# magnusgrandin/ca-lanczos

Hardware: AMD Instinct MI355X
Metric: CA-Lanczos outer-iters/sec (n~10M, s=8) (higher is better)
Workload: dtype f64; 1 GPU; lap3d_215: 7-pt 3-D 215x..., n=9938375, nnz=69291275; s=8, basis=newton, orth=local, parallelism=row-slab x1, normalize=auto, comm=none, halo=none

## Files before the change

ca_lanczos_amd/csrc/blockorth.cpp:

```cpp
#include <algorithm>
#include <chrono>
#include <cstdlib>
#include <cmath>
#include <vector>

#include "cal_internal.hpp"
#include "comm.hpp"
#include "dense.hpp"

namespace cal {

static Panel panel_slice(const Panel& P, int c0, int nc) {
    Panel out = panel();
    int base = 0;
    for (int s = 0; s < P.nseg; ++s) {
        const int lo = std::max(c0, base), hi = std::min(c0 + nc, base + P.ncol[s]);
        if (hi > lo) panel_add(out, P.ptr[s] + (int64_t)(lo - base) * P.ld[s], P.ld[s], hi - lo);
        base += P.ncol[s];
    }
    return out;
}

static PanelOut panel_out_slice(const PanelOut& P, int c0, int nc) {
    PanelOut out{};
// ... 297 lines not shown
    auto coeffs_b = [&](bool* sh2) -> int {
        std::vector<double> Gp = G1, Rb((size_t)m * m), Rbi((size_t)m * m);
        for (int j = 0; j < m; ++j)
            for (int i = 0; i < m; ++i) {
                double s = 0.0;
                for (int k = 0; k < w; ++k) s += C3[k + (size_t)i * w] * C3[k + (size_t)j * w];
                Gp[i + (size_t)j * m] -= s;
            }
        if (!chol_or_shift(m, Gp.data(), ng, Rb.data(), sh2))
            return set_error(c, CAL_ERR_NUMERIC, "block orthogonalisation: second Cholesky failed");
        dense::tri_inv_upper(m, Rb.data(), m, Rbi.data(), m);
        std::fill(M2.begin(), M2.end(), 0.0);
        for (int j = 0; j < m; ++j) {
            for (int i = 0; i < w; ++i) {
                double s = 0.0;
                for (int k = 0; k <= j; ++k) s += C3[i + (size_t)k * w] * Rbi[k + (size_t)j * m];
                M2[i + (size_t)j * (w + m)] = -s;
            }
            for (int i = 0; i < m; ++i) M2[w + i + (size_t)j * (w + m)] = Rbi[i + (size_t)j * m];
        }
        for (int j = 0; j < m; ++j)
            for (int i = 0; i < w; ++i) {
                double s = 0.0;
                for (int k = 0; k <= j; ++k) s += C3[i + (size_t)k * w] * Racc[k + (size_t)j * m];
                Ctot[i + (size_t)j * w] += s;
            }
        std::vector<double> Rn((size_t)m * m, 0.0);
        dense::matmul(m, m, m, Rb.data(), m, Racc.data(), m, Rn.data(), m);
        for (int j = 0; j < m; ++j)
            for (int i = j + 1; i < m; ++i) Rn[i + (size_t)j * m] = 0.0;
        Racc = Rn;
        return 0;
    };
    if (fast && !sh) {
        double G16[256], e16[16];
        CAL_TRY(rowapply_host(c, n, W, M1.data(), m, Qout, 2, w, G16, e16));
        unpack(G16, e16, G1, C3);
        bool sh2 = false;
        CAL_TRY(coeffs_b(&sh2));
        CAL_TRY(rowapply_host(c, n, W, M1.data(), m, Qout, 3, w, nullptr, nullptr, M2.data()));
        std::copy(Racc.begin(), Racc.end(), R);
        *shifted = *shifted || sh2;
        return 0;
    }
    CAL_TRY(grams(W, M1, G1, C3, false));
    const int passes = sh ? 2 : 1;
    for (int p = 0; p < passes; ++p) {
        bool sh2 = false;
        CAL_TRY(coeffs_b(&sh2));
        sh = sh || sh2;
        const bool more = p + 1 < passes;
        CAL_TRY(grams(P2, M2, G1, C3, !more));
    }
    std::copy(Racc.begin(), Racc.end(), R);
    *shifted = *shifted || sh;
    return 0;
}

static bool orth_device_ok(cal_ctx* c, const Panel& Qp, const Panel& X) {
    const int w = Qp.total, m = X.total, nq = w < 8 ? w : 8;
    return c->orth_coef_device && m >= 1 && w <= 9 && nq + m <= 16 && Qp.nseg + X.nseg <= kMaxSeg &&
           rowapply_ok(w + m, m, true, w);
}

constexpr int kSweepResMax = 3;
constexpr int64_t kSweepResBudget = ((int64_t)256 << 20) / 32 * 29;
static int sweep_policy(cal_ctx* c, int64_t n, int w, int m) {
    int res = -1;
    if (w == 9 && m == 8 && !c->pbw.want && !test_switch("CAL_TEST_SWEEP_STREAM_OFF")) {
        const int64_t r = std::min<int64_t>(std::min(m, kSweepResMax), kSweepResBudget / (8 * std::max<int64_t>(n, 1)));
        const bool large = (int64_t)n * 8 * (w + m) > ((int64_t)256 << 20);
        if ((large && c->sweep_x_fresh) || test_switch("CAL_TEST_SWEEP_STREAM_ON")) res = (int)r;
    }
#ifdef CAL_TEST_HOOKS
    c->test_sweep_res = res;
#endif
    return res;
}

#ifdef CAL_TEST_HOOKS
}
extern "C" int cal_test_sweep_policy(cal_ctx* c) { return c ? c->test_sweep_res : -2; }
extern "C" int cal_test_sweep_coef(cal_ctx* c) { return c ? c->test_sweep_coef : -2; }
namespace cal {
#endif

static int wait_published(cal_ctx* c, const unsigned long long* h_seq, unsigned long long seq) {
    const auto t0 = std::chrono::steady_clock::now();
    for (uint64_t spin = 1;; ++spin) {
        if (__atomic_load_n(h_seq, __ATOMIC_ACQUIRE) == seq) return 0;
        if ((spin & 4095) == 0 && std::chrono::steady_clock::now() - t0 > std::chrono::seconds(2)) {
            CAL_HIP(c, hipStreamSynchronize(c->stream));
            if (__atomic_load_n(h_seq, __ATOMIC_ACQUIRE) == seq) return 0;
            return set_error(c, CAL_ERR_HIP, "block orthogonalisation: result never published");
        }
        __builtin_ia32_pause();
    }
}

static int orth_device(cal_ctx* c, int64_t n, const Panel& Qp, const Panel& X, bool doreorth, const PanelOut& Qout,
                       double* Rq, double* R, bool* reorth, int p1_blocks = 0) {
    const int w = Qp.total, m = X.total, nq = w < 8 ? w : 8, wp = w + m;
    const int WP = rowapply_wpmax(wp), MO = rowapply_mout(m);
    const Panel W = panel_concat(Qp, X);
    const int res = sweep_policy(c, n, w, m);
    const int csrc = test_switch("CAL_TEST_SWEEP_COEF_LDS") ? 0 : (test_switch("CAL_TEST_SWEEP_COEF_SCALAR") ? 1 : -1);
#ifdef CAL_TEST_HOOKS
    c->test_sweep_coef = rowapply_coef(wp, m, 2, n, csrc);
#endif
    CAL_TRY(ensure_red(c, 4096));
    double* d_tile = c->d_red;
    double* d_st = c->d_red + 1024;
    double* d_mbuf = c->d_red + 2048;
    double* d_out = c->d_red + 3072;
#ifdef CAL_TEST_HOOKS
    CAL_HIP(c, hipMemsetAsync(c->d_red, 0xFF, 4096 * sizeof(double), c->stream));
#endif
    const double* gate = test_switch("CAL_TEST_NO_PASSB_GATE") ? nullptr : d_out + 512;
    const int64_t rg_cap = (int64_t)n * 8 * 17 <= ((int64_t)160 << 20) ? kRowGramBlocks / 2 : kRowGramBlocks;
    int64_t blocks = std::max<int64_t>(1, std::min<int64_t>((n + 255) / 256, rg_cap));
    CAL_TRY(ensure_partial(c, (size_t)blocks * 272));
    ColList ct{};
    if (p1_blocks > 0 && w == 0) {
    } else {
        p1_blocks = 0;
        const Panel T = panel_concat(panel_slice(W, 0, nq), X);
        const int nt = T.total;
        for (int cc = 0; cc < 16; ++cc) ct.p[cc] = panel_slice(T, cc < nt ? cc : nt - 1, 1).ptr[0];
        ct.p[16] = w == 9 ? panel_slice(Qp, 8, 1).ptr[0] : ct.p[0];
        const int t = timer_begin(c, 1, 8.0 * n * (nt + (w == 9 ? 1 : 0)));
        CAL_HIP(c, launch_rowgram(ct, nt, w == 9, n, (int)blocks, c->d_partial, c->stream, res));
        timer_end(c, t);
    }
    CAL_TRY(ensure_pub(c));
    const unsigned long long seq = ++c->pub_seq;
    double* h_out = c->h_pub;
    unsigned long long* h_seq = reinterpret_cast<unsigned long long*>(c->h_pub + 516);
    unsigned long long* d_seq = reinterpret_cast<unsigned long long*>(c->d_pub + 516);
    auto coef = [&](int phase, int dore) -> int {
        const int np = phase == 0 && p1_blocks > 0 ? p1_blocks : (int)blocks;
        CAL_HIP_OTHER(c, launch_reduce(c->d_partial, np, 272, d_tile, c->stream));
        CAL_TRY(allreduce_sum(c, d_tile, 272));
        CAL_HIP_OTHER(c, launch_orth_coef(phase, d_tile, d_st, d_mbuf, d_out, w, m, WP, MO, dore,
                                    phase == 1 ? c->d_pub : nullptr, d_seq, seq, c->stream));
        return 0;
    };
    CAL_TRY(coef(0, doreorth ? 1 : 0));
    ColList cw{};
    OutList ol{};
    for (int cc = 0; cc < 17; ++cc) cw.p[cc] = panel_slice(W, cc < wp ? cc : wp - 1, 1).ptr[0];
    for (int j = 0; j < 16; ++j) ol.p[j] = panel_out_slice(Qout, j < m ? j : 0, 1).ptr[0];
    {
        const int t = timer_begin(c, 1, 8.0 * n * wp);
        CAL_HIP(c, launch_rowapply(cw, d_mbuf, wp, m, ol, 2, w, n, (int)blocks, c->d_partial, c->stream, nullptr,
                                   res, csrc));
        timer_end(c, t);
    }
    CAL_TRY(coef(1, 0));
    const bool pbw = c->pbw.want && w == 9 && m == 8 && WP == 17 && MO == 8 &&
                     passb_wide_tiles(c->pbw.qold.total) <= kPassbWideMaxTiles && Qp.nseg == 1 &&
                     c->pbw.qold.nseg <= 1;
    c->pbw.want = false;
    c->pbw.ready = false;
    if (pbw) {
        const int ntw = passb_wide_tiles(c->pbw.qold.total);
        const size_t ent = (size_t)128 * ntw;
        const int pblocks = (int)std::max<int64_t>(1, std::min<int64_t>((n + 255) / 256, kRowGramBlocks));
        CAL_TRY(ensure_partial(c, (size_t)pblocks * ent));
        if (ent > c->pbw.cap) {
            if (c->pbw.d) CAL_HIP(c, hipFree(c->pbw.d));
            if (c->pbw.h) CAL_HIP(c, hipHostFree(c->pbw.h));
            c->pbw.d = c->pbw.h = nullptr;
            c->pbw.cap = 0;
            const size_t cap = (size_t)128 * kPassbWideMaxTiles;
            CAL_HIP(c, scratch_malloc((void**)&c->pbw.d, cap * sizeof(double)));
            CAL_HIP(c, hipHostMalloc((void**)&c->pbw.h, cap * sizeof(double), hipHostMallocDefault));
            c->pbw.cap = cap;
        }
        if (!c->pbw.ev) CAL_HIP(c, hipEventCreateWithFlags(&c->pbw.ev, hipEventDisableTiming));
        const int t = timer_begin(c, 2, 8.0 * n * (wp + m + c->pbw.qold.total));
        CAL_HIP(c, launch_passb_wide(cw, d_mbuf, ol, c->pbw.qold, n, pblocks, c->d_partial, gate, c->stream));
        timer_end(c, t);
        CAL_HIP_OTHER(c, launch_reduce(c->d_partial, pblocks, (int64_t)ent, c->pbw.d, c->stream));
        CAL_TRY(allreduce_sum(c, c->pbw.d, (int64_t)ent));
        CAL_HIP_OTHER(c, hipMemcpyAsync(c->pbw.h, c->pbw.d, ent * sizeof(double), hipMemcpyDeviceToHost, c->stream));
        CAL_HIP(c, hipEventRecord(c->pbw.ev, c->stream));
        c->pbw.ntw = ntw;
    } else {
        const int t = timer_begin(c, 2, 8.0 * n * (wp + m));
        CAL_HIP(c, launch_rowapply(cw, d_mbuf, wp, m, ol, 3, w, n, (int)((n + 255) / 256), c->d_partial, c->stream,
                                   gate, res, csrc));
        timer_end(c, t);
    }
    if (c->pre_wait) {
        auto hook = std::move(c->pre_wait);
        c->pre_wait = nullptr;
        CAL_TRY(hook());
    }
    CAL_TRY(wait_published(c, h_seq, seq));
    if (h_out[512] != 0.0 || h_out[513] != 0.0) return 1;
    c->pbw.ready = pbw;
    std::copy(h_out, h_out + (size_t)m * m, R);
    std::copy(h_out + 256, h_out + 256 + (size_t)w * m, Rq);
    *reorth = h_out[514] != 0.0;
    return 0;
}

int normalize_dev(cal_ctx* c, int64_t n, const Panel& X, const PanelOut& Qout, double* R, double tol, int* rank,
                  bool* shifted, int p1_blocks) {
    const int m = X.total;
    if (use_tsqr(c, m, c->tier1)) {
        CAL_TRY(tsqr_dev(c, n, X, nullptr, m, Qout, R));
        if (shifted) *shifted = false;
        if (rank) *rank = rank_from_R(m, R, tol);
        return 0;
    }
    auto via_tsqr = [&]() -> int {
        CAL_TRY(tsqr_dev(c, n, X, nullptr, m, Qout, R));
        if (shifted) *shifted = false;
        if (rank) *rank = rank_from_R(m, R, tol);
        return 0;
    };
    if (m > 16 && tsqr_ok(m)) return via_tsqr();
    if (m < 1 || m > 16) return set_error(c, CAL_ERR_ARG, "normalize: 1..32 columns supported");
    if (orth_device_ok(c, panel(), X)) {
        bool ro = false;
        const int st = orth_device(c, n, panel(), X, false, Qout, nullptr, R, &ro, p1_blocks);
        CAL_TRY(st);
        if (st == 0) {
            if (shifted) *shifted = false;
            if (rank) *rank = rank_from_R(m, R, tol);
            return 0;
        }
        c->orth_redone = true;
        if (c->normalize_kind != 2) return via_tsqr();
    }
    std::vector<double> G((size_t)m * m), Mz((size_t)m * m, 0.0), Ctot;
    if (X.nseg <= kMaxSeg) {
// ... 706 lines not shown
```

ca_lanczos_amd/csrc/cal_internal.hpp:

```cpp
#pragma once

#include <hip/hip_runtime.h>
#include <rocprofiler-sdk-roctx/roctx.h>

#include <cstdint>
#include <cstdlib>
#include <functional>
#include <string>
#include <vector>

#include "../../include/calanczos.h"

struct RoctxRange {
    explicit RoctxRange(const char* msg) { roctxRangePushA(msg); }
    ~RoctxRange() { roctxRangePop(); }
    RoctxRange(const RoctxRange&) = delete;
    RoctxRange& operator=(const RoctxRange&) = delete;
};

namespace cal {

constexpr int kMaxSeg = 4;

struct Panel {
// ... 147 lines not shown
    bool ds_neg1 = false;
    uint8_t* ds_rowmask = nullptr;
    uint32_t* ds_wavemask = nullptr;
    double* ds_diag = nullptr;
    double* ds_gsum = nullptr;
    double* ds_dprod = nullptr;
    bool shared = false;
    int64_t n_half = 0;
    bool herm = false;
    double* vim = nullptr;
    int* dpos = nullptr;
    int dpos_state = 0;
    int64_t dpos_missing = 0, dpos_dup = 0;
    std::vector<int> peers;
    std::vector<int64_t> recv_off;
    std::vector<int64_t> recv_cnt;
    std::vector<int64_t> send_off;
    std::vector<int64_t> send_cnt;
    int* send_idx = nullptr;
    int64_t send_total = 0;
    double* send_buf = nullptr;
};

struct Comm;
struct LanczosState;
struct PropState;
struct StdLanczosState;

hipError_t launch_spmv(const SpmvArgs& a, hipStream_t st);
hipError_t launch_spmv_stacked(const SpmvArgs& a, const double* vim, int64_t n_half, hipStream_t st);
hipError_t launch_spmv_pat(const PatArgs& a, hipStream_t st);
int spmv_lanczos_blocks(const SpmvArgs& a);
int spmv_pat_lanczos_blocks(const PatArgs& a);
hipError_t launch_spmv_dsplit(const PatArgs& a, hipStream_t st);
int spmv_dsplit_blocks(const PatArgs& a);
struct GramPlan {
    int nta;
    int blocks;
    int64_t entries;
};
GramPlan gram_plan(int wa, int wb, int64_t n);
hipError_t launch_gram(const Panel& A, const Panel& B, int64_t n, const GramPlan& pl, double* partial,
                       hipStream_t st);
bool gram_bb_ok(int wa, int wb);
hipError_t launch_gram_bb(const Panel& A, const Panel& B, int64_t n, const GramPlan& pl, double* partial,
                          hipStream_t st);
struct ApplyPlan {
    int nty;
    int run;
    int blocks;
    bool gram;
    bool gramp;
    size_t lds_bytes;
    int64_t entries;
};
ApplyPlan apply_plan(int wp, int wy, int64_t n, bool gram, int wq);
int apply_rows_max_wy(int wp);
bool apply_rows_ok(int wp, int wy);
bool apply_gram_ok(int wp, int wy, int wq);
int apply_gram_blocks(int64_t n);
hipError_t launch_apply_gram(const Panel& P, const double* dM, int wp, int wy, const PanelOut& Y, const Panel& Qn,
                             int64_t n, double* partial, hipStream_t st);
bool apply_selfgram_ok(int wp, int wy);
hipError_t launch_apply_selfgram(const Panel& P, const double* dM, int wp, int wy, const PanelOut& Y, int64_t n,
                                 double* partial, int* blocks, hipStream_t st);
hipError_t launch_apply(const Panel& P, const double* dM, int wp, int wy, const PanelOut& Y, bool store,
                        int wq, int64_t n, const ApplyPlan& pl, double* partial, hipStream_t st);
hipError_t launch_reduce(const double* partial, int nparts, int64_t nent, double* out, hipStream_t st);
hipError_t launch_gram_wide(const double* Q, int64_t ld, int w, int64_t n, double* partial, hipStream_t st);
int gram_wide_entries(int w);
int gram_wide_blocks(int64_t n);
void gram_wide_entry(int w, int e, int* i, int* j);
hipError_t launch_tilegram(const Panel& T, const double* E, int64_t n, int blocks, double* partial, hipStream_t st);
int rowapply_wpmax(int wp);
int rowapply_mout(int m);
struct ColList {
    const double* p[17];
};
struct OutList {
    double* p[16];
};
hipError_t launch_rowapply(const ColList& P, const double* dM, int wp, int m, const OutList& Y, int kind, int wq,
                           int64_t n, int blocks, double* partial, hipStream_t st, const double* gate = nullptr,
                           int res = -1, int coef = -1);
int rowapply_coef(int wp, int m, int kind, int64_t n, int coef);
hipError_t launch_orth_coef(int phase, const double* tile, double* st, double* mbuf, double* out, int w, int m,
                            int WP, int MO, int doreorth, double* hout, unsigned long long* hseq,
                            unsigned long long seq, hipStream_t stream);
#ifndef CAL_ROWGRAM_BLOCKS
#define CAL_ROWGRAM_BLOCKS 1024
#endif
constexpr int kRowGramBlocks = CAL_ROWGRAM_BLOCKS;
hipError_t launch_rowgram(const ColList& P, int nt, bool has_extra, int64_t n, int blocks, double* partial,
                          hipStream_t st, int res = -1);
constexpr int kPassbWideMaxTiles = 12;
int passb_wide_tiles(int wold);
hipError_t launch_passb_wide(const ColList& P, const double* dM, const OutList& Y, const Panel& Qold, int64_t n,
                             int blocks, double* partial, const double* gate, hipStream_t st);
hipError_t launch_dot(const double* x, const double* y, int64_t n, double* partial, int blocks,
                      hipStream_t st);
int dot_blocks(int64_t n);
hipError_t launch_axpy_sub(double* y, const double* x, double a, int64_t n, hipStream_t st);
hipError_t launch_div(double* y, const double* x, double b, int64_t n, hipStream_t st);
hipError_t launch_form_projM(const double* G, int ldg, int w, int m, double* M, hipStream_t st);
hipError_t launch_normest_norms(double* x, const double* y, int64_t n, double* part, double* dst, hipStream_t st);
hipError_t launch_normest_norms_only(const double* x, const double* y, int64_t n, double* part, double* dst,
                                     hipStream_t st);
hipError_t launch_pro_step(double* r, const double* qprev, const double* pb_prev, const double* q, double* qnext,
                           int64_t n, double* part, double* d_alpha, double* d_beta2, hipStream_t st);
hipError_t launch_pro_tail(double* r, const double* q, double* qnext, int64_t n, const double* pa, int np, double* pb,
                           double* d_alpha, double* d_beta2, hipStream_t st);
hipError_t launch_axpy_sub_dev(double* y, const double* x, const double* pa, bool take_sqrt, int64_t n,
                               hipStream_t st);
hipError_t launch_div_sqrt(double* y, const double* x, const double* nn, int64_t n, hipStream_t st);
hipError_t launch_abs_rowsum(const int* rowptr, const double* val, int64_t n, double* y, hipStream_t st);
hipError_t launch_gather(double* dst, const double* src, const int* idx, int64_t cnt, hipStream_t st);
int gram_async(cal_ctx* c, int64_t n, const Panel& A, const Panel& B, double* d_dst, double* h_dst, int* ldc,
               double* part = nullptr, bool bb = false);
int spmv_pair_resid_blocks(const PatArgs& a);
hipError_t launch_spmv_pair_resid(const PatArgs& a, double lr, double* partial, hipStream_t st);
hipError_t launch_spmv_pair_resid_multi(const PatArgs& a, const double* X, int64_t ldx, const int* col,
                                        const double* lam, const int* out, int npr, double* partial,
                                        int64_t pstride, hipStream_t st);
int spmv_resid_pair_multi_dev(cal_ctx* c, const double* X, int64_t ldx, const int* col, const double* lam,
                              const int* out, int npr, double* partial, int64_t pstride);
int spmv_pair_resid_multi_blocks(const PatArgs& a);
int spmv_resid_pair_multi_blocks(cal_ctx* c);
bool apply_mt_ok(int wp, int wy);
hipError_t launch_apply_mt(const double* P, int64_t ldp, const double* dM, int wp, int wy, double* Y, int64_t ldy,
                           int64_t n, hipStream_t st);
int spmv_resid_pair_dev(cal_ctx* c, const double* x, double lr, double* partial, int* blocks);
int spmv_resid_pair_blocks(cal_ctx* c);
hipError_t launch_spmv_resid(const SpmvArgs& a, const double* xi, double lr, double li, int64_t nrows,
                             double* partial, int blocks, hipStream_t st);

constexpr int kTsqrMaxCols = 33;
struct TsqrCols {
    const double* p[kTsqrMaxCols];
};
struct TsqrQ {
    double* p[32];
};
struct TsqrLevelArgs {
    int64_t rows = 0;
    int m = 0;
    int wp = 0;
    const double* M = nullptr;
    const double* in = nullptr;
    double* out = nullptr;
    const double* S = nullptr;
    const double* M2 = nullptr;
    int w2 = 0;
    double* V = nullptr;
    double* tb = nullptr;
};
int tsqr_mm(int m);
int tsqr_tile_rows(int m);
bool tsqr_form_ok(int wp, int m);
hipError_t launch_tsqr(bool down, int src, const TsqrLevelArgs& a, const TsqrCols& P, const TsqrQ& Q,
                       hipStream_t st);


constexpr double kFoldTol = 1e-14;
struct FoldArgs {
    int64_t n = 0;
    double tol = kFoldTol;
    int m = 0, w = 0, nblk = 0, n0 = 0, nlev = 0;
    int nu[3] = {0, 0, 0};
    const double* C = nullptr;
    const double* flags = nullptr;
    const double* K = nullptr;
    double *V0 = nullptr, *tb0 = nullptr, *R0 = nullptr;
    double* Vu[3] = {nullptr, nullptr, nullptr};
    double* Ru[3] = {nullptr, nullptr, nullptr};
    double* Mu[3] = {nullptr, nullptr, nullptr};
    double* Rroot_m = nullptr;
    double* partial = nullptr;
// ... 78 lines not shown
    hipEvent_t a, b;
    double bytes;
};

struct cal_ctx {
    int device = 0;
    hipStream_t stream = nullptr;
    hipStream_t aux_stream = nullptr;
    std::string err;
    cal::DevMatrix A;
    bool has_A = false;
    uint64_t A_gen = 0;
    int64_t stat_spmv_rows = 0;

    double* d_partial = nullptr;
    size_t partial_cap = 0;
    double* d_red = nullptr;
    double* h_red = nullptr;
    size_t red_cap = 0;
    double* d_small = nullptr;
    double* h_small = nullptr;
    size_t small_cap = 0;
    bool small_pending = false;
    double* d_scratch = nullptr;
    size_t scratch_cap = 0;

    double* d_work = nullptr;
    int work_cols = 0;
    int64_t work_ld = 0;

    cal::LanczosState* lz = nullptr;
    cal::PropState* prop = nullptr;
    cal::StdLanczosState* slz = nullptr;
    cal::Comm* comm = nullptr;

    bool timing = false;
    std::vector<CalTimerRec> timers;
    std::vector<hipEvent_t> event_pool;

    int spmv_format = 0;
    int mpk_depth_req = 8;
    int powers_launches = 0;
    int powers_schedule = -1;
    bool orth_coef_device = true;
    std::function<int()> pre_wait;
    struct {
        bool want = false, ready = false;
        cal::Panel qold{};
        int ntw = 0;
        double* d = nullptr;
        double* h = nullptr;
        size_t cap = 0;
        hipEvent_t ev = nullptr;
    } pbw;
    bool orth_redone = false;
    bool sweep_x_fresh = false;
    hipEvent_t orth_event = nullptr;
    double* h_pub = nullptr;
    double* d_pub = nullptr;
    unsigned long long pub_seq = 0;
    int normalize_kind = 0;
    bool tier1 = false;
    double* d_tsqr = nullptr;
    size_t tsqr_cap = 0;
    double* d_tsqrv = nullptr;
    size_t tsqrv_cap = 0;
    double* d_zbuf = nullptr;
    size_t zbuf_cap = 0;
    double* d_fold = nullptr;
    size_t fold_cap = 0;
    long fold_runs = 0, fold_declined = 0;
    double fold_last_est = 0.0;
    double fold_tol = cal::kFoldTol;
    hipStream_t nest_stream = nullptr;
    hipEvent_t nest_event = nullptr;
    double* d_nest = nullptr;
    double* h_nest = nullptr;
    size_t nest_cap = 0;
    hipGraphExec_t nest_exec[2] = {nullptr, nullptr};
    std::vector<int64_t> nest_key[2];
    std::vector<double> test_R1;
    int test_sweep_res = -2;
    int test_sweep_coef = -2;
};

namespace cal {

int set_error(cal_ctx* c, int code, const std::string& msg);
int hip_fail(cal_ctx* c, hipError_t e, const char* what);

#define CAL_HIP(ctx, expr)                                  \
    do {                                                    \
        hipError_t _e = (expr);                             \
        if (_e != hipSuccess) return cal::hip_fail((ctx), _e, #expr); \
    } while (0)
#define CAL_HIP_OTHER(ctx, expr)                                            \
    do {                                                                    \
        const int _t = cal::timer_begin((ctx), 3);                          \
        hipError_t _e = (expr);                                             \
        cal::timer_end((ctx), _t);                                          \
        if (_e != hipSuccess) return cal::hip_fail((ctx), _e, #expr);       \
    } while (0)
#define CAL_TRY(expr)             \
    do {                          \
        int _s = (expr);          \
        if (_s < 0) return _s;    \
    } while (0)

constexpr int kPubDoubles = 520;
int ensure_pub(cal_ctx* c);

int upload_matrix(cal_ctx* c, int64_t n_rows, int64_t ext_off, int64_t n_local, int64_t n_global, int64_t row0,
                  int64_t nghost, int64_t lpad, int64_t rext, const std::vector<int>& rowptr,
                  const std::vector<int>& col, const double* val);
int upload_matrix_shared(cal_ctx* c, int64_t n, const std::vector<int>& rowptr, const std::vector<int>& col,
                         const double* val, const double* vim = nullptr);
int shared_refuses(cal_ctx* c, const char* what);
int shared_format_only_stacked(cal_ctx* c, const char* who);
int spmv_range(cal_ctx* c, int64_t o, int64_t len, const double* x, double* y, int mode, double shift, double im2,
               const double* xprev);
int powers_dev(cal_ctx* c, int s, const double* q, double* const* Y, const double* shift, const double* im2,
               const double* const* xprev);
int halo_exchange_deep(cal_ctx* c, double* x, int d, hipStream_t st);
inline hipError_t copy_cols(cal_ctx* c, double* dst, const double* src, int64_t ld, int64_t n, int m) {
    if (n <= 0 || m <= 0) return hipSuccess;
    return hipMemcpy2DAsync(dst, ld * sizeof(double), src, ld * sizeof(double), n * sizeof(double), m,
                            hipMemcpyDeviceToDevice, c->stream);
}
inline double* vcol(const cal_ctx* c, double* base, int64_t j) { return base + j * c->A.ld + c->A.lpad; }
inline bool test_switch(const char* name) {
#ifdef CAL_TEST_HOOKS
    return std::getenv(name) != nullptr;
#else
    (void)name;
    return false;
#endif
}
hipError_t scratch_malloc(void** p, size_t bytes);
int ensure_partial(cal_ctx* c, size_t doubles);
int ensure_scratch(cal_ctx* c, size_t doubles);
int ensure_red(cal_ctx* c, size_t doubles);
int ensure_small(cal_ctx* c, size_t doubles);
int ensure_work(cal_ctx* c, int cols, int64_t ld);
double* work_col(cal_ctx* c, int j);

int timer_begin(cal_ctx* c, int kind, double bytes = 0.0);
int timer_begin_on(cal_ctx* c, int kind, hipStream_t st);
void timer_end_on(cal_ctx* c, int idx, hipStream_t st);
void timer_end(cal_ctx* c, int idx);

struct LanczosBegin {
    const double* r_host = nullptr;
    const double* r_dev = nullptr;
    double rr = -1.0;
    const double* shifts = nullptr;
    int nshifts = 0;
    bool prologue_cgs = true;
    bool reuse = false;
};
int lanczos_begin(cal_ctx* c, const LanczosBegin& in, int s, int max_outer, const char* basis, const char* orth);
int lanczos_step(cal_ctx* c, int diagnostics);
struct LanczosView {
    int s, k, ldt;
    const double* T;
    const double* b;
    const double* Q;
// ... 52 lines not shown
```

ca_lanczos_amd/csrc/kernels.hip:

```cpp
#include <algorithm>
#include <cstdio>
#include <cstdlib>
#include <type_traits>
#include <utility>

#include "cal_internal.hpp"

namespace cal {

typedef double d4 __attribute__((ext_vector_type(4)));
typedef double d2 __attribute__((ext_vector_type(2)));

constexpr int kSpmvThreads = 256;
constexpr int kSpmvNnz = 2048;
#ifndef CAL_RESID_PLANES
#define CAL_RESID_PLANES 32
#endif
constexpr int kResidPlanes = CAL_RESID_PLANES;

template <typename T, typename PT>
__device__ __forceinline__ T* seg_col(const PT P, int c) {
    T* res = P.ptr[0];
    int base = 0;
#pragma unroll
// ... 3012 lines not shown
#pragma unroll
                    for (int j = 0; j < MOUT; ++j) asm volatile("" : "+v"(y2[j])::"memory");
                }
                const double src = c < WPMAX ? p[c < WPMAX ? c : 0] : y[c >= WPMAX ? c - WPMAX : 0];
                const double* row = c < WPMAX ? M2p + c * MOUT : M2y + (c - WPMAX) * MOUT;
                double mrow[MOUT];
#pragma unroll
                for (int j = 0; j < MOUT; j += 2) {
                    const d2 t = *reinterpret_cast<const d2*>(&row[j]);
                    mrow[j] = t[0];
                    if (j + 1 < MOUT) mrow[j + 1] = t[1];
                }
#pragma unroll
                for (int j = 0; j < MOUT; ++j) y2[j] = __builtin_fma(src, mrow[j], y2[j]);
            }
#pragma unroll
            for (int j = 0; j < MOUT; ++j) y[j] = y2[j];
        }
        if (APPLY && STORE && in) {
#pragma unroll
            for (int j = 0; j < MOUT; ++j) {
                if (j < m) {
                    if constexpr (NTS) __builtin_nontemporal_store(y[j], &yc[j][r]);
                    else yc[j][r] = y[j];
                }
            }
        }
        if (GRAM) {
            double* trow = tile + tid * TLD;
            if (APPLY) {
#pragma unroll
                for (int c = 0; c < 8; ++c)
                    if (c < nq) trow[c] = p[c < WPMAX ? c : 0];
#pragma unroll
                for (int j = 0; j < MOUT; ++j)
                    if (j < m) trow[nq + j] = y[j];
                trow[16] = has_ext ? p[8 < WPMAX ? 8 : 0] : 0.0;
            } else {
#pragma unroll
                for (int c = 0; c < 16; ++c)
                    if (c < m) trow[c] = p[c < WPMAX ? c : 0];
                trow[16] = wq > 0 ? p[16 < WPMAX ? 16 : 0] : 0.0;
            }
            wave_lds_sync();
#pragma unroll
            for (int k = 0; k < 16; ++k) {
                const int row = wave * 64 + 4 * k + g;
                const double a = tile[row * TLD + c16];
                acc = mfma64(a, a, acc);
                eacc = eacc + tile[row * TLD + 16] * a;
            }
            wave_lds_sync();
        }
    }
    if (GRAM) __syncthreads();
    if (GRAM) {
        if (wave > 0) {
#pragma unroll
            for (int r = 0; r < 4; ++r) red[((wave - 1) * 64 + lane) * 5 + r] = acc[r];
            red[((wave - 1) * 64 + lane) * 5 + 4] = eacc;
        }
        __syncthreads();
        if (wave == 0) {
            const int64_t nb = gridDim.x;
            double* out = partial + blockIdx.x;
#pragma unroll
            for (int r = 0; r < 4; ++r) {
                double v = acc[r];
                v = v + red[(0 * 64 + lane) * 5 + r];
                v = v + red[(1 * 64 + lane) * 5 + r];
                v = v + red[(2 * 64 + lane) * 5 + r];
                out[(int64_t)(c16 * 16 + g + 4 * r) * nb] = v;
            }
            double e = eacc;
            e = e + red[(0 * 64 + lane) * 5 + 4];
            e = e + red[(1 * 64 + lane) * 5 + 4];
            e = e + red[(2 * 64 + lane) * 5 + 4];
            const double e1 = __shfl(e, c16 + 16, 64), e2 = __shfl(e, c16 + 32, 64), e3 = __shfl(e, c16 + 48, 64);
            if (g == 0) out[(int64_t)(256 + c16) * nb] = ((e + e1) + e2) + e3;
        }
    }
}

#ifndef CAL_SWEEP_RESIDENT
#define CAL_SWEEP_RESIDENT -2
#endif
static_assert(CAL_SWEEP_RESIDENT >= -2 && CAL_SWEEP_RESIDENT <= 3, "CAL_SWEEP_RESIDENT: -2, -1 or 0..3");
static int sweep_res(int res) {
    if (res < 0 || res > 3 || CAL_SWEEP_RESIDENT == -1) return -1;
    return CAL_SWEEP_RESIDENT >= 0 ? CAL_SWEEP_RESIDENT : res;
}
#define CAL_RES_SWITCH(res, LAUNCH) \
    switch (res) {                  \
        case 0: LAUNCH(0); break;   \
        case 1: LAUNCH(1); break;   \
        case 2: LAUNCH(2); break;   \
        case 3: LAUNCH(3); break;   \
        default: LAUNCH(-1); break; \
    }

int rowapply_wpmax(int wp) { return wp <= 5 ? 5 : (wp <= 9 ? 9 : (wp <= 17 ? 17 : 0)); }
int rowapply_mout(int m) { return m <= 4 ? 4 : (m <= 8 ? 8 : (m <= 16 ? 16 : 0)); }

#ifndef CAL_SWEEP_COEF
#define CAL_SWEEP_COEF -1
#endif
static_assert(CAL_SWEEP_COEF >= -1 && CAL_SWEEP_COEF <= 1, "CAL_SWEEP_COEF: -1, 0 or 1");
#ifndef CAL_SWEEP_COEF_KINDS
#define CAL_SWEEP_COEF_KINDS 3
#endif
int rowapply_coef(int wp, int m, int kind, int64_t n, int coef) {
    if (rowapply_wpmax(wp) != 17 || rowapply_mout(m) != 8 || (kind != 2 && kind != 3)) return 0;
    if (coef < 0) coef = CAL_SWEEP_COEF;
    if (coef >= 0) return coef ? 1 : 0;
    if (!((CAL_SWEEP_COEF_KINDS >> (kind - 2)) & 1)) return 0;
    return (int64_t)n * 8 * (wp + m) > ((int64_t)256 << 20) ? 1 : 0;
}

hipError_t launch_rowapply(const ColList& P, const double* dM, int wp, int m, const OutList& Y, int kind, int wq,
                           int64_t n, int blocks, double* partial, hipStream_t st, const double* gate, int res,
                           int coef) {
    const int WP = rowapply_wpmax(wp), MO = rowapply_mout(m);
    coef = rowapply_coef(wp, m, kind, n, coef);
    dim3 g(blocks), b(256);
    const bool nts = (int64_t)n * 8 * (wp + m) > ((int64_t)256 << 20);
    res = wp == 17 && m == 8 && (kind == 2 || kind == 3) ? sweep_res(res) : -1;
#define CAL_RA_PASSA(R) \
    hipLaunchKernelGGL((k_rowapply<17, 8, true, true, false, false, false, R>), g, b, 0, st, P, dM, wp, m, Y, wq, n, \
                       partial, gate)
#define CAL_RA_PASSB(R) \
    hipLaunchKernelGGL((k_rowapply<17, 8, false, true, true, true, true, R>), g, b, 0, st, P, dM, wp, m, Y, wq, n, \
                       partial, gate)
#define CAL_RA_PASSA_S(R) \
    hipLaunchKernelGGL((k_rowapply<17, 8, true, true, false, false, false, R, 1>), g, b, 0, st, P, dM, wp, m, Y, wq, n, \
                       partial, gate)
#define CAL_RA_PASSB_S(R) \
    hipLaunchKernelGGL((k_rowapply<17, 8, false, true, true, true, true, R, 1>), g, b, 0, st, P, dM, wp, m, Y, wq, n, \
                       partial, gate)
    if (coef) {
        if (kind == 2) {
            CAL_RES_SWITCH(res, CAL_RA_PASSA_S)
        } else if (res >= 0 || nts) {
            CAL_RES_SWITCH(res, CAL_RA_PASSB_S)
        } else {
            hipLaunchKernelGGL((k_rowapply<17, 8, false, true, true, true, false, -1, 1>), g, b, 0, st, P, dM, wp, m, Y,
                               wq, n, partial, gate);
        }
        return hipGetLastError();
    }
    if (res >= 0) {
        if (kind == 2) {
            CAL_RES_SWITCH(res, CAL_RA_PASSA)
        } else {
            CAL_RES_SWITCH(res, CAL_RA_PASSB)
        }
        return hipGetLastError();
    }
#undef CAL_RA_PASSB_S
#undef CAL_RA_PASSA_S
#undef CAL_RA_PASSB
#undef CAL_RA_PASSA
#define CAL_RA(W, MM, G, S, C) \
    hipLaunchKernelGGL((k_rowapply<W, MM, G, true, S, C>), g, b, 0, st, P, dM, wp, m, Y, wq, n, partial, gate)
#define CAL_RA_NT(W, MM) \
    hipLaunchKernelGGL((k_rowapply<W, MM, false, true, true, true, true>), g, b, 0, st, P, dM, wp, m, Y, wq, n, partial, \
                       gate)
#define CAL_RA_SHAPE(W, MM)                                  \
    case W * 100 + MM:                                       \
        switch (kind) {                                      \
            case 0: CAL_RA(W, MM, false, true, false); break; \
            case 1: CAL_RA(W, MM, true, true, false); break;  \
            case 2: CAL_RA(W, MM, true, false, false); break; \
            default:                                         \
                if (nts) CAL_RA_NT(W, MM);                   \
                else CAL_RA(W, MM, false, true, true);       \
                break;                                       \
        }                                                    \
        break;
    switch (WP * 100 + MO) {
        CAL_RA_SHAPE(5, 4)
        CAL_RA_SHAPE(5, 8)
        CAL_RA_SHAPE(9, 4)
        CAL_RA_SHAPE(9, 8)
        CAL_RA_SHAPE(9, 16)
        CAL_RA_SHAPE(17, 4)
        CAL_RA_SHAPE(17, 8)
        case 1716:
            if (kind != 0) return hipErrorInvalidValue;
            CAL_RA(17, 16, false, true, false);
            break;
        default: return hipErrorInvalidValue;
    }
#undef CAL_RA_SHAPE
#undef CAL_RA_NT
#undef CAL_RA
    return hipGetLastError();
}

template <int NTW, bool NTS>
__global__ __launch_bounds__(256) void k_passb_wide(ColList P, const double* __restrict__ M, OutList Y,
                                                    const double* __restrict__ qold, int64_t ldq, int wold,
                                                    int64_t n, double* __restrict__ partial,
                                                    const double* __restrict__ gate) {
    constexpr int WPMAX = 17, MOUT = 8, WQ = 9;
    constexpr int MSZ = WPMAX * MOUT * 2 + MOUT * MOUT;
    constexpr int TLD = 17;
    constexpr int WTILE = 64 * TLD;
    constexpr int RT = 4;
    constexpr int LDSZ = 4 * WTILE;
// ... 88 lines not shown
        wave_lds_sync();
#pragma unroll
        for (int t = 0; t < NTW; ++t) {
            if (t == 0) {
#pragma unroll
                for (int c = 0; c < 16; ++c) tw[lane * TLD + c] = c < WQ ? p[c < WQ ? c : 0] : y[c >= WQ ? c - WQ : 0];
            } else {
#pragma unroll
                for (int c = 0; c < 16; ++c) tw[lane * TLD + c] = (t == 1 && c == 0) ? y[7] : nxt[c];
                if (t + 1 < NTW) load_old(t + 1);
            }
            wave_lds_sync();
#pragma unroll
            for (int kk = 0; kk < 16; ++kk) acc[t] = mfma64(tw[(4 * kk + g) * TLD + c16], bv[kk], acc[t]);
            wave_lds_sync();
        }
    }
    auto red = reinterpret_cast<double (*)[RT][64][4]>(lds);
    const int64_t nb = gridDim.x;
    double* out = partial + blockIdx.x;
#pragma unroll
    for (int t0 = 0; t0 < NTW; t0 += RT) {
        __syncthreads();
        if (wave > 0) {
#pragma unroll
            for (int t = t0; t < (t0 + RT < NTW ? t0 + RT : NTW); ++t)
#pragma unroll
                for (int q = 0; q < 4; ++q) red[wave - 1][t - t0][lane][q] = acc[t][q];
        }
        __syncthreads();
        if (wave == 0 && c16 < MOUT) {
#pragma unroll
            for (int t = t0; t < (t0 + RT < NTW ? t0 + RT : NTW); ++t)
#pragma unroll
                for (int q = 0; q < 4; ++q) {
                    double v = acc[t][q];
                    v = v + red[0][t - t0][lane][q];
                    v = v + red[1][t - t0][lane][q];
                    v = v + red[2][t - t0][lane][q];
                    const int a = 16 * t + g + 4 * q, j = c16;
                    out[(int64_t)(j * 16 * NTW + a) * nb] = v;
                }
        }
    }
}

int passb_wide_tiles(int wold) { return (9 + 8 + wold + 15) / 16; }

hipError_t launch_passb_wide(const ColList& P, const double* dM, const OutList& Y, const Panel& Qold, int64_t n,
                             int blocks, double* partial, const double* gate, hipStream_t st) {
    if (Qold.total > 0 && Qold.nseg != 1) return hipErrorInvalidValue;
    const int ntw = passb_wide_tiles(Qold.total);
    const double* qold = Qold.total > 0 ? Qold.ptr[0] : P.p[0];
    const int64_t ldq = Qold.total > 0 ? Qold.ld[0] : 0;
    const int wold = Qold.total;
    const bool nts = (int64_t)n * 8 * (17 + 8) > ((int64_t)256 << 20);
    dim3 g(blocks), b(256);
#define CAL_PBW(T)                                                                                              \
    case T:                                                                                                     \
        if (nts) hipLaunchKernelGGL((k_passb_wide<T, true>), g, b, 0, st, P, dM, Y, qold, ldq, wold, n, partial, \
                                    gate);                                                                      \
        else hipLaunchKernelGGL((k_passb_wide<T, false>), g, b, 0, st, P, dM, Y, qold, ldq, wold, n, partial, \
                                gate);                                                                          \
        break;
    switch (ntw) {
        CAL_PBW(2)
        CAL_PBW(3)
        CAL_PBW(4)
        CAL_PBW(5)
        CAL_PBW(6)
        CAL_PBW(7)
        CAL_PBW(8)
        CAL_PBW(9)
        CAL_PBW(10)
        CAL_PBW(11)
        CAL_PBW(12)
        default: return hipErrorInvalidValue;
    }
#undef CAL_PBW
    return hipGetLastError();
}

hipError_t launch_rowgram(const ColList& P, int nt, bool has_extra, int64_t n, int blocks, double* partial,
                          hipStream_t st, int res) {
    OutList none{};
    res = nt == 16 && has_extra ? sweep_res(res) : -1;
#define CAL_RG(R)                                                                                                   \
    hipLaunchKernelGGL((k_rowapply<17, 4, true, false, true, false, false, R>), dim3(blocks), dim3(256), 0, st, P, \
                       nullptr, 17, nt, none, has_extra ? 1 : 0, n, partial, nullptr)
    CAL_RES_SWITCH(res, CAL_RG)
#undef CAL_RG
    return hipGetLastError();
}


__global__ __launch_bounds__(256) void k_reduce(const double* __restrict__ part, int nparts,
                                                double* __restrict__ out) {
    __shared__ double ws[4];
    const int64_t e = blockIdx.x;
    const double* p = part + e * nparts;
    double s = 0.0;
    for (int i = threadIdx.x; i < nparts; i += 256) s = s + p[i];
    s = wave_sum(s);
    const int lane = threadIdx.x & 63, wave = threadIdx.x >> 6;
    if (lane == 0) ws[wave] = s;
    __syncthreads();
    if (threadIdx.x == 0) out[e] = ((ws[0] + ws[1]) + ws[2]) + ws[3];
}

hipError_t launch_reduce(const double* partial, int nparts, int64_t nent, double* out, hipStream_t st) {
    if (nent <= 0) return hipSuccess;
    hipLaunchKernelGGL(k_reduce, dim3((unsigned)nent), dim3(256), 0, st, partial, nparts, out);
    return hipGetLastError();
}

__global__ __launch_bounds__(256) void k_dot(const double* __restrict__ x, const double* __restrict__ y,
                                             int64_t n, double* __restrict__ partial) {
    __shared__ double ws[4];
    double s = 0.0;
    const int64_t stride = (int64_t)gridDim.x * 256;
    for (int64_t i = (int64_t)blockIdx.x * 256 + threadIdx.x; i < n; i += stride) s = s + x[i] * y[i];
    s = wave_sum(s);
    const int lane = threadIdx.x & 63, wave = threadIdx.x >> 6;
    if (lane == 0) ws[wave] = s;
    __syncthreads();
    if (threadIdx.x == 0) partial[blockIdx.x] = ((ws[0] + ws[1]) + ws[2]) + ws[3];
}

int dot_blocks(int64_t n) {
    int64_t b = (n + 255) / 256;
    if (b > 1024) b = 1024;
    if (b < 1) b = 1;
    return (int)b;
}

hipError_t launch_dot(const double* x, const double* y, int64_t n, double* partial, int blocks,
                      hipStream_t st) {
    hipLaunchKernelGGL(k_dot, dim3(blocks), dim3(256), 0, st, x, y, n, partial);
    return hipGetLastError();
}

__global__ __launch_bounds__(256) void k_axpy_sub(double* __restrict__ y, const double* __restrict__ x, double a,
                                                  int64_t n) {
    const int64_t stride = (int64_t)gridDim.x * 256;
    for (int64_t i = (int64_t)blockIdx.x * 256 + threadIdx.x; i < n; i += stride) {
        const double t = a * x[i];
        y[i] = y[i] - t;
    }
}

__global__ __launch_bounds__(256) void k_div(double* __restrict__ y, const double* __restrict__ x, double b,
                                             int64_t n) {
    const int64_t stride = (int64_t)gridDim.x * 256;
    for (int64_t i = (int64_t)blockIdx.x * 256 + threadIdx.x; i < n; i += stride) y[i] = x[i] / b;
}

__global__ __launch_bounds__(256) void k_gather(double* __restrict__ dst, const double* __restrict__ src,
                                                const int* __restrict__ idx, int64_t cnt) {
    const int64_t i = (int64_t)blockIdx.x * 256 + threadIdx.x;
    if (i < cnt) dst[i] = src[idx[i]];
}

static unsigned vec_blocks(int64_t n) {
    int64_t b = (n + 255) / 256;
    if (b > 4096) b = 4096;
    if (b < 1) b = 1;
    return (unsigned)b;
}

// ... 563 lines not shown
```

Before: 954.6 outer-iters/s.

## Add MFMA-based tiled Gram kernel for hot block-orth sweep passes

Introduces k_gramtile, which stages 17-column row tiles through LDS and accumulates the 16x16 Gram with MFMA f64 instructions plus a scalar extra column, replacing k_rowapply for the rowgram and pass-A apply in the w=9,m=8 large-n case. It also adds software prefetch of the next chunk's rows and a waves-per-EU hint. The aim is to cut the VALU FMA cost of the Gram reduction so the sweep stays bandwidth-bound. In exchange it adds LDS traffic and per-wave syncs, and changes the floating-point summation order.

```diff
diff --git a/ca_lanczos_amd/csrc/blockorth.cpp b/ca_lanczos_amd/csrc/blockorth.cpp
--- a/ca_lanczos_amd/csrc/blockorth.cpp
+++ b/ca_lanczos_amd/csrc/blockorth.cpp
@@ -403,6 +403,7 @@
 }
 extern "C" int cal_test_sweep_policy(cal_ctx* c) { return c ? c->test_sweep_res : -2; }
 extern "C" int cal_test_sweep_coef(cal_ctx* c) { return c ? c->test_sweep_coef : -2; }
+extern "C" int cal_test_sweep_tile(cal_ctx* c) { return c ? c->test_sweep_tile : -2; }
 namespace cal {
 #endif
 
@@ -426,8 +427,10 @@
     const Panel W = panel_concat(Qp, X);
     const int res = sweep_policy(c, n, w, m);
     const int csrc = test_switch("CAL_TEST_SWEEP_COEF_LDS") ? 0 : (test_switch("CAL_TEST_SWEEP_COEF_SCALAR") ? 1 : -1);
+    const int tsrc = test_switch("CAL_TEST_SWEEP_TILE_FULL") ? 0 : (test_switch("CAL_TEST_SWEEP_TILE_SMALL") ? 1 : -1);
 #ifdef CAL_TEST_HOOKS
     c->test_sweep_coef = rowapply_coef(wp, m, 2, n, csrc);
+    c->test_sweep_tile = sweep_tile(w == 9 && m == 8, n, tsrc);
 #endif
     CAL_TRY(ensure_red(c, 4096));
     double* d_tile = c->d_red;
@@ -450,7 +453,7 @@
         for (int cc = 0; cc < 16; ++cc) ct.p[cc] = panel_slice(T, cc < nt ? cc : nt - 1, 1).ptr[0];
         ct.p[16] = w == 9 ? panel_slice(Qp, 8, 1).ptr[0] : ct.p[0];
         const int t = timer_begin(c, 1, 8.0 * n * (nt + (w == 9 ? 1 : 0)));
-        CAL_HIP(c, launch_rowgram(ct, nt, w == 9, n, (int)blocks, c->d_partial, c->stream, res));
+        CAL_HIP(c, launch_rowgram(ct, nt, w == 9, n, (int)blocks, c->d_partial, c->stream, res, tsrc));
         timer_end(c, t);
     }
     CAL_TRY(ensure_pub(c));
@@ -474,7 +477,7 @@
     {
         const int t = timer_begin(c, 1, 8.0 * n * wp);
         CAL_HIP(c, launch_rowapply(cw, d_mbuf, wp, m, ol, 2, w, n, (int)blocks, c->d_partial, c->stream, nullptr,
-                                   res, csrc));
+                                   res, csrc, tsrc));
         timer_end(c, t);
     }
     CAL_TRY(coef(1, 0));
diff --git a/ca_lanczos_amd/csrc/cal_internal.hpp b/ca_lanczos_amd/csrc/cal_internal.hpp
--- a/ca_lanczos_amd/csrc/cal_internal.hpp
+++ b/ca_lanczos_amd/csrc/cal_internal.hpp
@@ -253,8 +253,9 @@
 };
 hipError_t launch_rowapply(const ColList& P, const double* dM, int wp, int m, const OutList& Y, int kind, int wq,
                            int64_t n, int blocks, double* partial, hipStream_t st, const double* gate = nullptr,
-                           int res = -1, int coef = -1);
+                           int res = -1, int coef = -1, int tile = -1);
 int rowapply_coef(int wp, int m, int kind, int64_t n, int coef);
+int sweep_tile(bool hot, int64_t n, int tile);
 hipError_t launch_orth_coef(int phase, const double* tile, double* st, double* mbuf, double* out, int w, int m,
                             int WP, int MO, int doreorth, double* hout, unsigned long long* hseq,
                             unsigned long long seq, hipStream_t stream);
@@ -263,7 +264,7 @@
 #endif
 constexpr int kRowGramBlocks = CAL_ROWGRAM_BLOCKS;
 hipError_t launch_rowgram(const ColList& P, int nt, bool has_extra, int64_t n, int blocks, double* partial,
-                          hipStream_t st, int res = -1);
+                          hipStream_t st, int res = -1, int tile = -1);
 constexpr int kPassbWideMaxTiles = 12;
 int passb_wide_tiles(int wold);
 hipError_t launch_passb_wide(const ColList& P, const double* dM, const OutList& Y, const Panel& Qold, int64_t n,
@@ -508,6 +509,7 @@
     std::vector<double> test_R1;
     int test_sweep_res = -2;
     int test_sweep_coef = -2;
+    int test_sweep_tile = -2;
 };
 
 namespace cal {
diff --git a/ca_lanczos_amd/csrc/kernels.hip b/ca_lanczos_amd/csrc/kernels.hip
--- a/ca_lanczos_amd/csrc/kernels.hip
+++ b/ca_lanczos_amd/csrc/kernels.hip
@@ -3118,6 +3118,128 @@
     }
 }
 
+template <int WPMAX, int RES, int XEND, int C = 0>
+__device__ __forceinline__ void tile_load_row(const double* const* pc, int64_t b, unsigned boff, double* dst) {
+    if constexpr (C < WPMAX) {
+        const uint64_t cb = reinterpret_cast<uint64_t>(pc[C] + b);
+        const uint64_t lo = (unsigned)__builtin_amdgcn_readfirstlane((unsigned)cb);
+        const uint64_t hi = (unsigned)__builtin_amdgcn_readfirstlane((unsigned)(cb >> 32));
+        typedef const __attribute__((address_space(1))) char* gbytes;
+        typedef const __attribute__((address_space(1))) double* gptr;
+        const gptr q = reinterpret_cast<gptr>(reinterpret_cast<gbytes>(hi << 32 | lo) + boff);
+        if constexpr (RES >= 0 && !(C >= XEND - RES && C < XEND)) dst[C] = __builtin_nontemporal_load(q);
+        else dst[C] = *q;
+        tile_load_row<WPMAX, RES, XEND, C + 1>(pc, b, boff, dst);
+    }
+}
+template <bool APPLY, int RES, int COEF, int TR, bool PF, int WPE>
+__global__ __launch_bounds__(256) __attribute__((amdgpu_waves_per_eu(WPE))) void k_gramtile(
+    ColList P, const double* __restrict__ M, int64_t n, double* __restrict__ partial) {
+    static_assert(TR == 16 || TR == 32 || TR == 64, "k_gramtile: 16, 32 or 64 tile rows per wave");
+    constexpr int TLD = 17, WPMAX = 17, MOUT = 8;
+    __shared__ double tile[4 * TR * TLD];
+    double* const red = tile;
+    __shared__ __attribute__((aligned(16))) double Ms[APPLY && !COEF ? WPMAX * MOUT : 2];
+    const double* const Mc = COEF ? M : Ms;
+    const int tid = threadIdx.x, lane = tid & 63, wave = tid >> 6;
+    const int c16 = lane & 15, g = lane >> 4;
+    if (APPLY && !COEF) {
+        for (int e = tid; e < WPMAX * MOUT; e += 256) Ms[e] = M[e];
+        __syncthreads();
+    }
+    d4 acc = d4{0.0, 0.0, 0.0, 0.0};
+    double eacc = 0.0;
+    const double* const* pc = P.p;
+    const int nch = (int)((n + 255) >> 8), nfull = (int)(n >> 8), cstride = gridDim.x;
+    const unsigned last = (unsigned)((n - 1) & 255);
+    double p[WPMAX];
+    auto load_rows = [&](int ci) {
+        const unsigned off = ci < nfull || (unsigned)tid < last ? (unsigned)tid : last;
+        tile_load_row<WPMAX, RES, APPLY ? WPMAX : 16>(pc, (int64_t)ci * 256, off * 8u, p);
+    };
+    double* const trow = tile + (wave * TR + lane % TR) * TLD;
+    const double* const twave = tile + (wave * TR + g) * TLD;
+    if (PF && (int)blockIdx.x < nch) load_rows(blockIdx.x);
+    for (int ci = blockIdx.x; ci < nch; ci += cstride) {
+        asm volatile("" ::: "memory");
+        const bool in = ci < nfull || (unsigned)tid <= last;
+        if (!PF) load_rows(ci);
+#pragma unroll
+        for (int c = 0; c < WPMAX; ++c) p[c] = in ? p[c] : 0.0;
+        double t[TLD];
+        if (APPLY) {
+            double y[MOUT];
+#pragma unroll
+            for (int j = 0; j < MOUT; ++j) y[j] = 0.0;
+#pragma unroll
+            for (int c = 0; c < WPMAX; ++c) {
+                if (!COEF || c % CAL_SWEEP_COEF_ROWS == 0) {
+#pragma unroll
+                    for (int j = 0; j < MOUT; ++j) asm volatile("" : "+v"(y[j])::"memory");
+                }
+                double mrow[MOUT];
+#pragma unroll
+                for (int j = 0; j < MOUT; j += 2) {
+                    const d2 v = *reinterpret_cast<const d2*>(&Mc[c * MOUT + j]);
+                    mrow[j] = v[0];
+                    mrow[j + 1] = v[1];
+                }
+#pragma unroll
+                for (int j = 0; j < MOUT; ++j) y[j] = __builtin_fma(p[c], mrow[j], y[j]);
+            }
+#pragma unroll
+            for (int c = 0; c < 8; ++c) t[c] = p[c];
+#pragma unroll
+            for (int j = 0; j < MOUT; ++j) t[8 + j] = y[j];
+            t[16] = p[8];
+        } else {
+#pragma unroll
+            for (int c = 0; c < TLD; ++c) t[c] = p[c];
+        }
+#pragma unroll
+        for (int h = 0; h < 64 / TR; ++h) {
+            if (lane / TR == h) {
+#pragma unroll
+                for (int c = 0; c < TLD; ++c) trow[c] = t[c];
+            }
+            if (PF && h == 64 / TR - 1 && ci + cstride < nch) load_rows(ci + cstride);
+            wave_lds_sync();
+#pragma unroll
+            for (int k = 0; k < TR / 4; ++k) {
+                const double a = twave[4 * k * TLD + c16];
+                acc = mfma64(a, a, acc);
+                eacc = eacc + twave[4 * k * TLD + 16] * a;
+            }
+            wave_lds_sync();
+        }
+    }
+    __syncthreads();
+    if (wave > 0) {
+#pragma unroll
+        for (int r = 0; r < 4; ++r) red[((wave - 1) * 64 + lane) * 5 + r] = acc[r];
+        red[((wave - 1) * 64 + lane) * 5 + 4] = eacc;
+    }
+    __syncthreads();
+    if (wave == 0) {
+        const int64_t nb = gridDim.x;
+        double* out = partial + blockIdx.x;
+#pragma unroll
+        for (int r = 0; r < 4; ++r) {
+            double v = acc[r];
+            v = v + red[(0 * 64 + lane) * 5 + r];
+            v = v + red[(1 * 64 + lane) * 5 + r];
+            v = v + red[(2 * 64 + lane) * 5 + r];
+            out[(int64_t)(c16 * 16 + g + 4 * r) * nb] = v;
+        }
+        double e = eacc;
+        e = e + red[(0 * 64 + lane) * 5 + 4];
+        e = e + red[(1 * 64 + lane) * 5 + 4];
+        e = e + red[(2 * 64 + lane) * 5 + 4];
+        const double e1 = __shfl(e, c16 + 16, 64), e2 = __shfl(e, c16 + 32, 64), e3 = __shfl(e, c16 + 48, 64);
+        if (g == 0) out[(int64_t)(256 + c16) * nb] = ((e + e1) + e2) + e3;
+    }
+}
+
 #ifndef CAL_SWEEP_RESIDENT
 #define CAL_SWEEP_RESIDENT -2
 #endif
@@ -3153,14 +3275,51 @@
     return (int64_t)n * 8 * (wp + m) > ((int64_t)256 << 20) ? 1 : 0;
 }
 
+#ifndef CAL_SWEEP_TILE
+#define CAL_SWEEP_TILE -1
+#endif
+static_assert(CAL_SWEEP_TILE >= -1 && CAL_SWEEP_TILE <= 1, "CAL_SWEEP_TILE: -1, 0 or 1");
+#ifndef CAL_SWEEP_TILE_ROWS
+#define CAL_SWEEP_TILE_ROWS 64
+#endif
+#ifndef CAL_SWEEP_TILE_PF_A
+#define CAL_SWEEP_TILE_PF_A 1
+#endif
+#ifndef CAL_SWEEP_TILE_WPE
+#define CAL_SWEEP_TILE_WPE (CAL_SWEEP_TILE_ROWS == 64 ? 4 : 5)
+#endif
+int sweep_tile(bool hot, int64_t n, int tile) {
+    if (!hot || n < 1 || n > ((int64_t)1 << 37)) return 0;
+    if (tile < 0) tile = CAL_SWEEP_TILE;
+    if (tile >= 0) return tile ? CAL_SWEEP_TILE_ROWS : 0;
+    return (int64_t)n * 8 * (17 + 8) > ((int64_t)256 << 20) ? CAL_SWEEP_TILE_ROWS : 0;
+}
+
 hipError_t launch_rowapply(const ColList& P, const double* dM, int wp, int m, const OutList& Y, int kind, int wq,
                            int64_t n, int blocks, double* partial, hipStream_t st, const double* gate, int res,
-                           int coef) {
+                           int coef, int tile) {
     const int WP = rowapply_wpmax(wp), MO = rowapply_mout(m);
     coef = rowapply_coef(wp, m, kind, n, coef);
+    tile = sweep_tile(kind == 2 && wp == 17 && m == 8 && wq == 9, n, tile);
     dim3 g(blocks), b(256);
     const bool nts = (int64_t)n * 8 * (wp + m) > ((int64_t)256 << 20);
     res = wp == 17 && m == 8 && (kind == 2 || kind == 3) ? sweep_res(res) : -1;
+    if (tile) {
+#define CAL_GT_PASSA(R)                                                                                            \
+    hipLaunchKernelGGL((k_gramtile<true, R, 0, CAL_SWEEP_TILE_ROWS, CAL_SWEEP_TILE_PF_A != 0, CAL_SWEEP_TILE_WPE>), g, b, \
+                       0, st, P, dM, n, partial)
+#define CAL_GT_PASSA_S(R)                                                                                          \
+    hipLaunchKernelGGL((k_gramtile<true, R, 1, CAL_SWEEP_TILE_ROWS, CAL_SWEEP_TILE_PF_A != 0, CAL_SWEEP_TILE_WPE>), g, b, \
+                       0, st, P, dM, n, partial)
+        if (coef) {
+            CAL_RES_SWITCH(res, CAL_GT_PASSA_S)
+        } else {
+            CAL_RES_SWITCH(res, CAL_GT_PASSA)
+        }
+#undef CAL_GT_PASSA_S
+#undef CAL_GT_PASSA
+        return hipGetLastError();
+    }
 #define CAL_RA_PASSA(R) \
     hipLaunchKernelGGL((k_rowapply<17, 8, true, true, false, false, false, R>), g, b, 0, st, P, dM, wp, m, Y, wq, n, \
                        partial, gate)
@@ -3415,9 +3574,17 @@
 }
 
 hipError_t launch_rowgram(const ColList& P, int nt, bool has_extra, int64_t n, int blocks, double* partial,
-                          hipStream_t st, int res) {
+                          hipStream_t st, int res, int tile) {
     OutList none{};
     res = nt == 16 && has_extra ? sweep_res(res) : -1;
+    if (sweep_tile(nt == 16 && has_extra, n, tile)) {
+#define CAL_GT_P1(R)                                                                                             \
+    hipLaunchKernelGGL((k_gramtile<false, R, 0, CAL_SWEEP_TILE_ROWS, true, CAL_SWEEP_TILE_WPE>), dim3(blocks), \
+                       dim3(256), 0, st, P, nullptr, n, partial)
+        CAL_RES_SWITCH(res, CAL_GT_P1)
+#undef CAL_GT_P1
+        return hipGetLastError();
+    }
 #define CAL_RG(R)                                                                                                   \
     hipLaunchKernelGGL((k_rowapply<17, 4, true, false, true, false, false, R>), dim3(blocks), dim3(256), 0, st, P, \
                        nullptr, 17, nt, none, has_extra ? 1 : 0, n, partial, nullptr)
```

Result: no change. 952.7 outer-iters/s (-0.2%).
